# lajoiepy/cslam

Hardware: AMD Instinct MI355X
Metric: keyframes/sec (extract+match) on 100kx4096-D bank (higher is better)
Workload: dtype f32

## Files before the change

cslam_amd/csrc/conv_stem_direct_h.hip:

```cpp
#include <stdlib.h>
#include <type_traits>
#include <hip/hip_fp16.h>
#include "common.h"
#include "pairs.h"
#include "direct_dev.h"

typedef float f32x4 __attribute__((ext_vector_type(4)));
typedef unsigned u32x4 __attribute__((ext_vector_type(4)));
typedef _Float16 f16x8 __attribute__((ext_vector_type(8)));

#define SD_IW 20
#define SD_IMG (12 * SD_IW * 3)
#define SD_T9 (20 * 17)
#define SD_IMGB (SD_IMG + SD_T9)
#define SD_LDS (2 * DPATCH_BYTES + 2 * SD_IMGB * 4)

struct StemDirectArgs {
    const float *x0; const unsigned *w1; const float *b1; const float *sumw; float inv_sw1;
    const f16x8 *w2; const float *bias; float inv_sw2;
    int B, H, W, gxb, gyb, nblk;
    const unsigned *amax_in; unsigned *amax_out; float *y;
};

#ifdef CSLAM_ABLATIONS
__device__ unsigned long long *sd_prof = nullptr;
extern "C" __attribute__((visibility("default"))) int cslam_debug_sd_prof_dev(void *d_buf) {
    unsigned long long *q = (unsigned long long *)d_buf;
    return hipMemcpyToSymbol(HIP_SYMBOL(sd_prof), &q, sizeof(q)) == hipSuccess ? 0 : -2;
}
#define SD_PROF 1
#else
#define SD_PROF 0
#endif

template <bool POOL, int DBG = 0>
__global__ __launch_bounds__(256, 1) void conv_stem_direct_h_kernel(StemDirectArgs p) {
    extern __shared__ __attribute__((aligned(16))) char sd_smem[];
    const int tid = threadIdx.x;
    const int lane = tid & 63;
    const int wave = __builtin_amdgcn_readfirstlane(tid >> 6);
    const int gq = lane >> 4, l15 = lane & 15;
    unsigned *const s_img_all = (unsigned *)(sd_smem + 2 * DPATCH_BYTES);

    const float a0 = fminf(fmaxf(__uint_as_float(*p.amax_in), 1e-30f), 1e30f);
    int e_;
    (void)frexpf(16384.0f / a0, &e_);
    const float s1 = ldexpf(1.0f, e_ - 1);
    const float inv1 = p.inv_sw1 / s1;
    float bound = 0.0f;
    for (int c = 0; c < 64; ++c) bound = fmaxf(bound, fabsf(p.b1 ? p.b1[c] : 0.0f) + a0 * p.sumw[c]);
    bound = fminf(fmaxf(bound, 1e-30f), 1e30f);
    (void)frexpf(32752.0f / bound, &e_);
    const float sx = ldexpf(1.0f, e_ - 1);
    const float inv2 = p.inv_sw2 / sx;

    const DirectPart part = direct_partition(p.nblk);
    const int n_mine = part.n_mine;
    if (n_mine <= 0) return;

    f16x8 wr[9][2][2];
#pragma unroll
    for (int tap = 0; tap < 9; ++tap)
#pragma unroll
        for (int ks = 0; ks < 2; ++ks)
#pragma unroll
            for (int hl = 0; hl < 2; ++hl) {
                wr[tap][ks][hl] = p.w2[(((wave * 9 + tap) * 2 + ks) * 2 + hl) * 64 + lane];
                asm volatile("" : "+a"(wr[tap][ks][hl]));
            }
    const u32x4 w1h = ((const u32x4 *)p.w1)[(wave * 2 + 0) * 64 + lane], w1l = ((const u32x4 *)p.w1)[(wave * 2 + 1) * 64 + lane];
    const f16x8 W1h = __builtin_bit_cast(f16x8, w1h), W1l = __builtin_bit_cast(f16x8, w1l);
    const float k1 = inv1 * sx;
    float b1s[4];
#pragma unroll
    for (int r = 0; r < 4; ++r) b1s[r] = (p.b1 ? p.b1[16 * wave + 4 * gq + r] : 0.0f) * sx;
    float4 bv2;
    bv2 = p.bias ? *(const float4 *)(p.bias + 16 * wave + 4 * gq) : make_float4(0.f, 0.f, 0.f, 0.f);

    int e_dst[3], e_rc[3];
#pragma unroll
    for (int j = 0; j < 3; ++j) {
        const int e = j * 256 + tid;
        const int ci = (e >= 240) + (e >= 480);
        const int rem = e - 240 * ci;
        const int r = (rem * 3277) >> 16, c = rem - 20 * r;
        e_dst[j] = e < SD_IMG ? (r * SD_IW + c) * 3 + ci : -1;
        e_rc[j] = (ci << 16) | (r << 8) | c;
    }
    typedef DirectBlk Blk;
    auto decode_blk = [&](int bi) { return direct_decode_blk(part, bi, p.gxb, p.gyb); };
    float raw[3];
    auto img_load = [&](const Blk &b) {
#pragma unroll
        for (int j = 0; j < 3; ++j) {
            const int ci = e_rc[j] >> 16, r = (e_rc[j] >> 8) & 255, c = e_rc[j] & 255;
            const int gy = b.by * 8 - 2 + r, gx = b.bx * 16 - 2 + c;
            const bool in = (e_dst[j] >= 0) & (gy >= 0) & (gy < p.H) & (gx >= 0) & (gx < p.W);
            raw[j] = in ? p.x0[((int64_t)(b.img * 3 + ci) * p.H + gy) * p.W + gx] : 0.0f;
        }
    };
    auto img_store = [&](unsigned *s_img) {
#pragma unroll
        for (int j = 0; j < 3; ++j)
            if (e_dst[j] >= 0) {
                const unsigned v = pack_pair(raw[j] * s1);
                s_img[e_dst[j]] = v;
                if ((e_rc[j] >> 16) == 2) s_img[SD_IMG + (e_rc[j] & 255) * 17 + ((e_rc[j] >> 8) & 255)] = v;
            }
    };

    int c1_src[12], c1_dst[12];
#pragma unroll
    for (int t = 0; t < 12; ++t) {
        int pp = 16 * t + l15;
        pp = pp < DPATCH_NPIX ? pp : DPATCH_NPIX - 1;
        const int pr = (pp * 3641) >> 16, pc = pp - 18 * pr;
        c1_src[t] = (gq < 3 ? ((pr + gq) * SD_IW + pc) * 3 : SD_IMG + (pc + 2) * 17 + pr) * 4;
        c1_dst[t] = DPATCH_OFF(pr, pc, 2 * wave + (gq >> 1), gq & 1);
    }
    for (int i = tid; i < 2 * 20 * 5; i += 256)
        s_img_all[(i / 100) * SD_IMGB + SD_IMG + ((i % 100) / 5) * 17 + 12 + (i % 5)] = 0u;
    unsigned pk[2][8];
    auto conv1_read = [&](int g, const unsigned *s_img) {
#pragma unroll
        for (int i = 0; i < 2; ++i) {
            const unsigned *ib = (const unsigned *)((const char *)s_img + c1_src[2 * g + i]);
#pragma unroll
            for (int j = 0; j < 8; ++j) pk[i][j] = ib[j];
        }
    };
    f32x4 c1[2];
    float c1v[2][4];
    auto conv1_piece = [&](int g, int piece, const Blk &b, char *patch) {
        const int i = piece & 1;
        if (piece < 2) {
            u32x4 ah, al;
#pragma unroll
            for (int d = 0; d < 4; ++d) {
                ah[d] = __builtin_amdgcn_perm(pk[i][2 * d + 1], pk[i][2 * d], 0x05040100u);
                al[d] = __builtin_amdgcn_perm(pk[i][2 * d + 1], pk[i][2 * d], 0x07060302u);
            }
            const f16x8 Ph = __builtin_bit_cast(f16x8, ah), Pl = __builtin_bit_cast(f16x8, al);
            c1[i] = __builtin_amdgcn_mfma_f32_16x16x32_f16(W1l, Ph, (f32x4)(0.0f), 0, 0, 0);
            c1[i] = __builtin_amdgcn_mfma_f32_16x16x32_f16(W1h, Pl, c1[i], 0, 0, 0);
            c1[i] = __builtin_amdgcn_mfma_f32_16x16x32_f16(W1h, Ph, c1[i], 0, 0, 0);
            asm volatile("" : "+v"(c1[i]));
            return;
        }
        if (piece < 4) {
#pragma unroll
            for (int r = 0; r < 4; ++r) c1v[i][r] = fmaxf(c1[i][r] * k1 + b1s[r], 0.0f);
            return;
        }
        const __half2 h01 = __floats2half2_rn(c1v[i][0], c1v[i][1]), h23 = __floats2half2_rn(c1v[i][2], c1v[i][3]);
        const float d0 = sub_half<0>(c1v[i][0], h01), d1 = sub_half<1>(c1v[i][1], h01);
        const float d2 = sub_half<0>(c1v[i][2], h23), d3 = sub_half<1>(c1v[i][3], h23);
        const __half2 l01 = __floats2half2_rn(d0, d1), l23 = __floats2half2_rn(d2, d3);
        if ((DBG & 16) == 0 && (2 * g + i < 11 || l15 < 4)) {
            char *d = patch + c1_dst[2 * g + i];
            *(uint2 *)d = make_uint2(*(const unsigned *)&h01, *(const unsigned *)&h23);
            *(uint2 *)(d + 128) = make_uint2(*(const unsigned *)&l01, *(const unsigned *)&l23);
        }
    };
    auto border_fixup = [&](const Blk &b, char *patch) {
        const int gy0 = b.by * 8 - 1, gx0 = b.bx * 16 - 1;
        if ((gy0 >= 0) & (gy0 + 10 <= p.H) & (gx0 >= 0) & (gx0 + 18 <= p.W)) return;
#pragma unroll
        for (int k = 0; k < 3; ++k) {
            const int pp = lane + 64 * k;
            const int pr = (pp * 3641) >> 16, pc = pp - 18 * pr;
            const int gy = gy0 + pr, gx = gx0 + pc;
            if (pp < DPATCH_NPIX && !((gy >= 0) & (gy < p.H) & (gx >= 0) & (gx < p.W))) {
                char *d = patch + pr * DPATCH_RP + pc * DPATCH_PP;
                const int c0 = ((2 * wave) ^ DPATCH_SWZ(pc)) << 4, c1_ = ((2 * wave + 1) ^ DPATCH_SWZ(pc)) << 4;
                *(uint4 *)(d + c0) = make_uint4(0u, 0u, 0u, 0u); *(uint4 *)(d + c1_) = make_uint4(0u, 0u, 0u, 0u);
                *(uint4 *)(d + 128 + c0) = make_uint4(0u, 0u, 0u, 0u); *(uint4 *)(d + 128 + c1_) = make_uint4(0u, 0u, 0u, 0u);
            }
        }
    };

    float my_amax = 0.0f;
    const int Ho = POOL ? p.H >> 1 : p.H, Wo = POOL ? p.W >> 1 : p.W;
    f32x4 eacc[8];
    Blk ecb = {0, 0, 0};
    bool e_ok = false;
    auto epi_piece = [&](int k) {
        const __amdgpu_buffer_rsrc_t rsY = buf_rsrc((const char *)(p.y + (int64_t)ecb.img * Ho * Wo * 64), (int64_t)Ho * Wo * 256, RSRC_LIM16);
        const int ox = ecb.bx * 16 + l15;
        const int ch_off = (16 * wave + 4 * gq) * 4;
        if (POOL) {
            const int py = ecb.by * 4 + k;
            float4 v;
            v.x = max_f32_xor1(max_f32(eacc[2 * k][0], eacc[2 * k + 1][0])); v.y = max_f32_xor1(max_f32(eacc[2 * k][1], eacc[2 * k + 1][1]));
            v.z = max_f32_xor1(max_f32(eacc[2 * k][2], eacc[2 * k + 1][2])); v.w = max_f32_xor1(max_f32(eacc[2 * k][3], eacc[2 * k + 1][3]));
            v.x = fmaxf(v.x * inv2 + bv2.x, 0.0f); v.y = fmaxf(v.y * inv2 + bv2.y, 0.0f);
            v.z = fmaxf(v.z * inv2 + bv2.z, 0.0f); v.w = fmaxf(v.w * inv2 + bv2.w, 0.0f);
            const bool store = e_ok & ((l15 & 1) == 0) & ((ox >> 1) < Wo) & (py < Ho);
            float m = max_f32(max_f32(v.x, v.y), max_f32(v.z, v.w));
            int off = (py * Wo + (ox >> 1)) * 256 + ch_off;
            asm volatile("" : "+v"(m), "+v"(off));
            my_amax = max_f32(my_amax, store ? m : 0.0f);
            u32x4 bits;
            bits.x = __float_as_uint(v.x); bits.y = __float_as_uint(v.y); bits.z = __float_as_uint(v.z); bits.w = __float_as_uint(v.w);
            if (!(DBG & 4)) __builtin_amdgcn_raw_buffer_store_b128(bits, rsY, store ? off : 0x7fffffff, 0, 0);
        } else {
#pragma unroll
            for (int r = 2 * k; r < 2 * k + 2; ++r) {
                const int oy = ecb.by * 8 + r;
                float4 v;
                v.x = fmaxf(eacc[r][0] * inv2 + bv2.x, 0.0f); v.y = fmaxf(eacc[r][1] * inv2 + bv2.y, 0.0f);
                v.z = fmaxf(eacc[r][2] * inv2 + bv2.z, 0.0f); v.w = fmaxf(eacc[r][3] * inv2 + bv2.w, 0.0f);
                const bool store = e_ok & (ox < p.W) & (oy < p.H);
                float m = max_f32(max_f32(v.x, v.y), max_f32(v.z, v.w));
                int off = (oy * p.W + ox) * 256 + ch_off;
                asm volatile("" : "+v"(m), "+v"(off));
                my_amax = max_f32(my_amax, store ? m : 0.0f);
                u32x4 bits;
                bits.x = __float_as_uint(v.x); bits.y = __float_as_uint(v.y); bits.z = __float_as_uint(v.z); bits.w = __float_as_uint(v.w);
                __builtin_amdgcn_raw_buffer_store_b128(bits, rsY, store ? off : 0x7fffffff, 0, 0);
            }
        }
    };

    f32x4 acc[8];
    int fr_off[3];
#pragma unroll
    for (int dx = 0; dx < 3; ++dx) fr_off[dx] = DPATCH_OFF(0, l15 + dx, gq, 0);
    f16x8 fh[3], fl[3];
    auto frag_read = [&](auto col_tag, auto r_tag, const char *patch) {
        constexpr int COL = decltype(col_tag)::value, R = decltype(r_tag)::value;
        constexpr int DX = COL >> 1, KS = COL & 1, SLOT = (R + COL) % 3;
        fh[SLOT] = *(const f16x8 *)(patch + fr_off[DX] + R * DPATCH_RP + KS * 64);
        fl[SLOT] = *(const f16x8 *)(patch + fr_off[DX] + R * DPATCH_RP + KS * 64 + 128);
    };
    auto rstep = [&](auto col_tag, auto r_tag, const char *patch, const unsigned *s_img, const Blk &nblk, char *npatch) {
        constexpr int COL = decltype(col_tag)::value, R = decltype(r_tag)::value;
        constexpr int DX = COL >> 1, KS = COL & 1, SLOT = (R + COL) % 3;
        if constexpr (DBG & 2) { }
        else if constexpr (R + 2 < 10) frag_read(col_tag, std::integral_constant<int, (R + 2) % 10>{}, patch);
        else if constexpr (COL < 5) frag_read(std::integral_constant<int, (COL + 1) % 6>{}, std::integral_constant<int, (R + 2) % 10>{}, patch);
        if constexpr (R == 0 && !(DBG & 1) && !(DBG & 8)) conv1_read(COL, s_img);
#pragma unroll
        for (int prod = 0; prod < 3; ++prod)
#pragma unroll
            for (int dy = 0; dy < 3; ++dy) {
                const int r = R - dy;
                if (r < 0 || r > 7) continue;
                const f16x8 a = prod == 2 ? wr[3 * dy + DX][KS][1] : wr[3 * dy + DX][KS][0];
                const f16x8 b = prod == 1 ? fl[SLOT] : fh[SLOT];
                acc[r] = __builtin_amdgcn_mfma_f32_16x16x32_f16(a, b, (COL == 0 && prod == 0 && dy == 0) ? (f32x4)(0.0f) : acc[r], 0, 0, 0);
            }
        if constexpr (R >= 2 && R <= 7 && !(DBG & 1)) conv1_piece(COL, R - 2, nblk, npatch);
        if constexpr (COL < 2 && (R == 1 || R == 8)) epi_piece(2 * COL + (R == 8 ? 1 : 0));
        __builtin_amdgcn_sched_group_barrier(0x100, R == 0 ? 18 : 2, 0);
        constexpr int NM = 3 * ((R < 2 ? R + 1 : 3) - (R > 7 ? R - 7 : 0)) + ((R == 2 || R == 3) ? 3 : 0);
#pragma unroll
        for (int m = 0; m < NM; ++m) {
            __builtin_amdgcn_sched_group_barrier(0x008, 1, 0);
            __builtin_amdgcn_sched_group_barrier(0x002, (COL < 2 && (R == 1 || R == 8)) ? 6 : 3, 0);
        }
        __builtin_amdgcn_sched_group_barrier(0x200, 2, 0);
        __builtin_amdgcn_sched_barrier(0);
    };
    auto edge = [&](auto col_tag, const char *patch, const unsigned *s_img) {
        constexpr int COL = decltype(col_tag)::value;
        constexpr int DX = COL >> 1, KS = COL & 1, SLOT = (9 + COL) % 3;
        constexpr int DX2 = (COL + 1) >> 1, KS2 = (COL + 1) & 1, SLOT2 = (COL + 1) % 3;
        if constexpr (!(DBG & 2)) frag_read(std::integral_constant<int, COL + 1>{}, std::integral_constant<int, 1>{}, patch);
        if constexpr (!(DBG & 1) && !(DBG & 8)) conv1_read(COL + 1, s_img);
#pragma unroll
        for (int prod = 0; prod < 3; ++prod) {
            acc[7] = __builtin_amdgcn_mfma_f32_16x16x32_f16(prod == 2 ? wr[6 + DX][KS][1] : wr[6 + DX][KS][0], prod == 1 ? fl[SLOT] : fh[SLOT], acc[7], 0, 0, 0);
            acc[0] = __builtin_amdgcn_mfma_f32_16x16x32_f16(prod == 2 ? wr[DX2][KS2][1] : wr[DX2][KS2][0], prod == 1 ? fl[SLOT2] : fh[SLOT2], acc[0], 0, 0, 0);
        }
        if constexpr (!(DBG & 2)) frag_read(std::integral_constant<int, COL + 1>{}, std::integral_constant<int, 2>{}, patch);
        __builtin_amdgcn_sched_group_barrier(0x100, 10, 0);
#pragma unroll
        for (int m = 0; m < 6; ++m) {
            __builtin_amdgcn_sched_group_barrier(0x008, 1, 0);
            __builtin_amdgcn_sched_group_barrier(0x002, 3, 0);
        }
        __builtin_amdgcn_sched_barrier(0);
    };
    auto column = [&](auto col_tag, const char *patch, const unsigned *s_img, const Blk &nblk, char *npatch) {
        constexpr int COL_ = decltype(col_tag)::value;
        if constexpr (COL_ == 0) rstep(col_tag, std::integral_constant<int, 0>{}, patch, s_img, nblk, npatch);
        rstep(col_tag, std::integral_constant<int, 1>{}, patch, s_img, nblk, npatch);
        rstep(col_tag, std::integral_constant<int, 2>{}, patch, s_img, nblk, npatch); rstep(col_tag, std::integral_constant<int, 3>{}, patch, s_img, nblk, npatch);
        rstep(col_tag, std::integral_constant<int, 4>{}, patch, s_img, nblk, npatch); rstep(col_tag, std::integral_constant<int, 5>{}, patch, s_img, nblk, npatch);
        rstep(col_tag, std::integral_constant<int, 6>{}, patch, s_img, nblk, npatch); rstep(col_tag, std::integral_constant<int, 7>{}, patch, s_img, nblk, npatch);
        rstep(col_tag, std::integral_constant<int, 8>{}, patch, s_img, nblk, npatch);
        if constexpr (COL_ == 5) rstep(col_tag, std::integral_constant<int, 9>{}, patch, s_img, nblk, npatch);
        else edge(col_tag, patch, s_img);
    };
#define SD_C(T) std::integral_constant<int, T>{}

    [[maybe_unused]] unsigned long long t_main = 0, t_epi = 0, t_bar = 0, t1 = 0, t2 = 0, t3 = 0;
    Blk cb = decode_blk(0);
    img_load(cb);
    img_store(s_img_all);
    Blk nb = decode_blk(1);
    img_load(nb);
    __syncthreads();
#pragma unroll
    for (int g = 0; g < 6; ++g) {
        conv1_read(g, s_img_all);
#pragma unroll
        for (int piece = 0; piece < 6; ++piece) conv1_piece(g, piece, cb, sd_smem);
        __builtin_amdgcn_sched_barrier(0);
    }
    border_fixup(cb, sd_smem);
    img_store(s_img_all + SD_IMGB);
    __syncthreads();
    for (int bi = 0; bi < n_mine; ++bi) {
        const int cur = bi & 1;
        const char *const patch = sd_smem + cur * DPATCH_BYTES;
        char *const npatch = sd_smem + (cur ^ 1) * DPATCH_BYTES;
        const unsigned *const s_img_next = s_img_all + (cur ^ 1) * SD_IMGB;
        const Blk nnb = decode_blk(bi + 2);
        img_load(nnb);
        if (SD_PROF) t1 = __builtin_amdgcn_s_memtime();
        frag_read(SD_C(0), SD_C(0), patch);
        frag_read(SD_C(0), SD_C(1), patch);
        column(SD_C(0), patch, s_img_next, nb, npatch); column(SD_C(1), patch, s_img_next, nb, npatch); column(SD_C(2), patch, s_img_next, nb, npatch);
        column(SD_C(3), patch, s_img_next, nb, npatch); column(SD_C(4), patch, s_img_next, nb, npatch); column(SD_C(5), patch, s_img_next, nb, npatch);
        if (!(DBG & 1)) border_fixup(nb, npatch);
        if (SD_PROF) { t2 = __builtin_amdgcn_s_memtime(); t_main += t2 - t1; }
        img_store(s_img_all + cur * SD_IMGB);
#pragma unroll
        for (int r = 0; r < 8; ++r) eacc[r] = acc[r];
        ecb = cb;
        e_ok = true;
        if (SD_PROF) { t3 = __builtin_amdgcn_s_memtime(); t_epi += t3 - t2; }
        __syncthreads();
        if (SD_PROF) t_bar += __builtin_amdgcn_s_memtime() - t3;
        cb = nb;
        nb = nnb;
    }
#pragma unroll
    for (int k = 0; k < 4; ++k) epi_piece(k);
#ifdef CSLAM_ABLATIONS
    if (sd_prof && blockIdx.x == 0 && tid == 0) { sd_prof[0] = t_main; sd_prof[1] = t_epi; sd_prof[2] = t_bar; sd_prof[3] = 0; sd_prof[4] = (unsigned long long)n_mine; }
#endif

    if (p.amax_out) {
        __syncthreads();
        amax_publish(my_amax, p.amax_out, sd_smem, tid, lane);
    }
}

CSLAM_API int cslam_conv_stem_direct_h_dev(const float *d_x0, const void *d_w1, const float *d_b1, const float *d_sumw, float inv_sw1,
                                           const void *d_w2r, const float *d_bias, float inv_sw2, int B, int H, int W, int pool,
                                           const unsigned *d_amax_x0, unsigned *d_amax_out, float *d_y, void *stream) {
    PTR_DEVICE(d_x0);
    ARG_CHECK(d_x0 && d_w1 && d_sumw && d_w2r && d_y && d_amax_x0, "NULL argument");
    ARG_CHECK(B >= 1 && H >= 1 && W >= 1, "empty map");
    ARG_CHECK(!pool || ((H % 2) == 0 && (W % 2) == 0), "pooling needs even H and W");
    ARG_CHECK(inv_sw1 > 0.0f && inv_sw2 > 0.0f, "scales must be positive");
    ARG_CHECK((int64_t)H * W * 256 < 0x7ffffff0ll, "one image's output map must stay below 2 GiB (32-bit buffer offsets)");
    StemDirectArgs a;
    a.x0 = d_x0; a.w1 = (const unsigned *)d_w1; a.b1 = d_b1; a.sumw = d_sumw; a.inv_sw1 = inv_sw1;
    a.w2 = (const f16x8 *)d_w2r; a.bias = d_bias; a.inv_sw2 = inv_sw2;
    a.B = B; a.H = H; a.W = W;
    a.gxb = (int)ceil_div64(W, 16); a.gyb = (int)ceil_div64(H, 8);
    const int64_t nblk = (int64_t)B * a.gxb * a.gyb;
    ARG_CHECK(nblk < (1ll << 30), "too many blocks for one launch");
    a.nblk = (int)nblk;
    a.amax_in = d_amax_x0; a.amax_out = d_amax_out; a.y = d_y;
    const int n_cu = cslam_cu_count();
    ARG_CHECK(n_cu > 0, "no HIP device");
    const int grid = (int)(nblk < n_cu ? nblk : n_cu);
    hipStream_t st = (hipStream_t)stream;
    const dim3 g(grid), b(256);
#ifdef CSLAM_ABLATIONS
    if (const char *e = getenv("CSLAM_SD_DBG")) {
        const int d = atoi(e);
        if (d == 1) return launch_lds<conv_stem_direct_h_kernel<true, 1>>(g, b, SD_LDS, st, a);
        if (d == 2) return launch_lds<conv_stem_direct_h_kernel<true, 2>>(g, b, SD_LDS, st, a);
        if (d == 3) return launch_lds<conv_stem_direct_h_kernel<true, 3>>(g, b, SD_LDS, st, a);
        if (d == 4) return launch_lds<conv_stem_direct_h_kernel<true, 4>>(g, b, SD_LDS, st, a);
        if (d == 7) return launch_lds<conv_stem_direct_h_kernel<true, 7>>(g, b, SD_LDS, st, a);
        if (d == 8) return launch_lds<conv_stem_direct_h_kernel<true, 8>>(g, b, SD_LDS, st, a);
        if (d == 16) return launch_lds<conv_stem_direct_h_kernel<true, 16>>(g, b, SD_LDS, st, a);
        if (d == 24) return launch_lds<conv_stem_direct_h_kernel<true, 24>>(g, b, SD_LDS, st, a);
    }
#endif
    if (pool) return launch_lds<conv_stem_direct_h_kernel<true>>(g, b, SD_LDS, st, a);
    return launch_lds<conv_stem_direct_h_kernel<false>>(g, b, SD_LDS, st, a);
}
```

cslam_amd/csrc/direct_dev.h:

```cpp
#pragma once
#include <hip/hip_fp16.h>
#include "common.h"
#include "pairs.h"

typedef unsigned dd_u32x2 __attribute__((ext_vector_type(2)));
typedef unsigned dd_u32x4 __attribute__((ext_vector_type(4)));
typedef float dd_f32x2 __attribute__((ext_vector_type(2)));

struct DirectPart { int wg_j, wg_per, blk_beg, blk_cnt, n_mine, half; };
template <bool PAIRS = false>
__device__ __forceinline__ DirectPart direct_partition(int nblk) {
    DirectPart q;
    const bool by_xcd = (gridDim.x & (PAIRS ? 15 : 7)) == 0;
    const int wg_xcd = by_xcd ? (int)blockIdx.x & 7 : 0, wg_raw = by_xcd ? (int)blockIdx.x >> 3 : (int)blockIdx.x;
    q.half = PAIRS ? wg_raw & 1 : 0;
    q.wg_j = PAIRS ? wg_raw >> 1 : wg_raw;
    q.wg_per = (by_xcd ? (int)gridDim.x >> 3 : (int)gridDim.x) >> (PAIRS ? 1 : 0);
    const int per_xcd = by_xcd ? (nblk + 7) >> 3 : nblk;
    q.blk_beg = wg_xcd * per_xcd;
    q.blk_cnt = min(per_xcd, nblk - q.blk_beg);
    q.n_mine = q.blk_cnt > q.wg_j ? (q.blk_cnt - q.wg_j + q.wg_per - 1) / q.wg_per : 0;
    return q;
}

struct DirectBlk { int img, by, bx; };
__device__ __forceinline__ DirectBlk direct_decode_blk(const DirectPart &q, int bi, int gxb, int gyb) {
    int blk = q.wg_j + bi * q.wg_per;
    blk = q.blk_beg + (blk < q.blk_cnt ? blk : q.blk_cnt - 1);
    const int per_img = gxb * gyb;
    DirectBlk b;
    b.img = blk / per_img;
    const int rem = blk - b.img * per_img;
    b.by = rem / gxb; b.bx = rem - b.by * gxb;
    return b;
}

__device__ __forceinline__ void amax_publish(float &my_amax, unsigned *amax_out, void *lds_slot, int tid, int lane) {
    unsigned *s_amax = (unsigned *)lds_slot;
    if (tid == 0) *s_amax = 0u;
    __syncthreads();
#pragma unroll
    for (int o = 32; o > 0; o >>= 1) my_amax = fmaxf(my_amax, __shfl_xor(my_amax, o, 64));
    if (lane == 0) atomicMax(s_amax, __float_as_uint(my_amax));
    __syncthreads();
    if (tid == 0 && *s_amax > *(volatile unsigned *)amax_out) atomicMax(amax_out, *s_amax);
}

constexpr int DPATCH_PP = 320;
constexpr int DPATCH_RP = 18 * DPATCH_PP;
constexpr int DPATCH_BYTES = 10 * DPATCH_RP;
constexpr int DPATCH_NPIX = 180;
constexpr int DPATCH_LO = 128;
#define DPATCH_SWZ(pc) (((pc) >> 1) & 3)
#define DPATCH_OFF(pr, pc, chunk, q) ((pr) * DPATCH_RP + (pc) * DPATCH_PP + (((chunk) ^ DPATCH_SWZ(pc)) << 4) + (q) * 8)

template <class Dst>
__device__ __forceinline__ void dpatch_split_store(dd_u32x4 v, float s, Dst dst) {
    dd_f32x2 w01 = dd_f32x2{__uint_as_float(v.x), __uint_as_float(v.y)} * dd_f32x2{s, s};
    dd_f32x2 w23 = dd_f32x2{__uint_as_float(v.z), __uint_as_float(v.w)} * dd_f32x2{s, s};
    asm("" : "+v"(w01), "+v"(w23));
    const __half2 h01 = __floats2half2_rn(w01[0], w01[1]), h23 = __floats2half2_rn(w23[0], w23[1]);
    const float d0 = sub_half<0>(w01[0], h01), d1 = sub_half<1>(w01[1], h01), d2 = sub_half<0>(w23[0], h23), d3 = sub_half<1>(w23[1], h23);
    const __half2 l01 = __floats2half2_rn(d0, d1), l23 = __floats2half2_rn(d2, d3);
    char *d = dst();
    *(uint2 *)d = make_uint2(*(const unsigned *)&h01, *(const unsigned *)&h23);
    *(uint2 *)(d + DPATCH_LO) = make_uint2(*(const unsigned *)&l01, *(const unsigned *)&l23);
// ... 14 lines not shown
```

cslam_amd/vpr/conv_kernels.py:

```python
import torch

from .. import _lib
from .heads import _p, _stream


def _po(t):
    return _p(t) if t is not None else None


def _out(B, C, H, W, pool, device):
    Ho, Wo = (H // 2, W // 2) if pool else (H, W)
    return torch.empty((B, C, Ho, Wo), dtype=torch.float32, device=device, memory_format=torch.channels_last)


def _amax_slot(x, slot, have=False):
    if not have and x.numel() % 4 == 0:
        _lib.check(_lib.load().cslam_absmax_dev(_p(x), x.numel(), _p(slot), _stream(x)))
    elif not have:
        slot.copy_(x.abs().max().reshape(1))
    return slot


def stem_pool_fits(Ho, Wo):
    return Ho % 8 == 0 and Wo % 16 == 0
# ... 100 lines not shown
    y = _out(B, 128, H, W, pool, x.device)
    _lib.check(fn(_p(x), _p(Wr[0]), _po(bias), B, H, W, Cin, 128, int(relu), int(pool), _p(amax_in), float(Wr[1]), _po(amax_out),
                  _p(y), _stream(x)))
    return y


def conv3x3_direct_r(x, Wr, bias, relu, pool, amax_in, amax_out=None):
    return _direct_r(_lib.load().cslam_conv3x3_direct_r_dev, x, Wr, bias, relu, pool, amax_in, amax_out)


def conv3x3_direct_r2(x, Wr2, bias, relu, pool, amax_in, amax_out=None):
    return _direct_r(_lib.load().cslam_conv3x3_direct_r2_dev, x, Wr2, bias, relu, pool, amax_in, amax_out)


def conv3x3_direct_r_pairs(x, Wr, bias, wl1, bmax, amax_in, bound_out, amax_out=None):
    x = x.contiguous(memory_format=torch.channels_last)
    B, Cin, H, W = x.shape
    y = torch.empty((B, H, W, 4, 2, 32), dtype=torch.float16, device=x.device)
    _lib.check(_lib.load().cslam_conv3x3_direct_r_pairs_dev(_p(x), _p(Wr[0]), _po(bias), B, H, W, Cin, 128, _p(amax_in), float(Wr[1]),
                                                            float(wl1), float(bmax), _po(amax_out), _p(bound_out), _p(y), _stream(x)))
    return y


def conv3x3_direct_hp(xp, shape, bound, Wd, bias, relu, pool, amax_out=None):
    B, Cin, H, W = shape
    W2, inv_sw = Wd
    Cout = W2.shape[1]
    y = _out(B, Cout, H, W, pool, xp.device)
    _lib.check(_lib.load().cslam_conv3x3_direct_hp_dev(_p(xp), _p(bound), _p(W2), _po(bias), B, H, W, Cin, Cout, int(relu), int(pool),
                                                       float(inv_sw), _po(amax_out), _p(y), _stream(xp)))
    return y


def conv_stem_direct_h(x0, stem, bias1, Wr, bias, pool, amax_x0, amax_out=None):
    B, C3, H, W = x0.shape
    assert C3 == 3 and x0.is_contiguous()
    y = _out(B, 64, H, W, pool, x0.device)
    _lib.check(_lib.load().cslam_conv_stem_direct_h_dev(
        _p(x0), _p(stem[0]), _po(bias1), _p(stem[2]), float(stem[1]), _p(Wr[0]), _po(bias), float(Wr[1]), B, H, W, int(pool),
        _p(amax_x0), _po(amax_out), _p(y), _stream(x0)))
    return y


def wino_stem64_h(x0, stem, bias1, Uh, bias, pool, amax_x0, amax_out=None):
    B, C3, H, W = x0.shape
    assert C3 == 3 and x0.is_contiguous() and Uh[0].shape[2] == 4
    y = _out(B, 64, H, W, pool, x0.device)
    _lib.check(_lib.load().cslam_wino4_stem_c64_h_dev(
        _p(x0), _p(stem[0]), _po(bias1), _p(stem[2]), float(stem[1]), _p(Uh[0]), _po(bias), B, H, W, int(pool), _p(amax_x0),
        float(Uh[1]), _po(amax_out), _p(y), _stream(x0)))
    return y


def _residual_like(residual, y):
    if residual is not None:
        residual = residual.contiguous(memory_format=torch.channels_last)
        assert residual.shape == y.shape
    return residual


def wino_fused64_h(x, Uh, bias, relu, pool, amax_in, amax_out=None, residual=None):
    B, _, H, W = x.shape
    Cout = Uh[0].shape[2] * 16
    y = _out(B, Cout, H, W, pool, x.device)
    residual = _residual_like(residual, y)
    _lib.check(_lib.load().cslam_wino4_fused_c64_h_dev(
        _p(x), _p(Uh[0]), _po(bias), _po(residual), B, H, W, Cout, int(relu), int(pool), _p(amax_in), float(Uh[1]), _po(amax_out),
        _p(y), _stream(x)))
    return y


def wino_fused64(x, Up, bias, relu, pool, residual=None):
    lib = _lib.load()
# ... 8 lines not shown
```

cslam_amd/vpr/winograd.py:

```python
import os

import torch
from torch import nn

from .. import _lib
from .conv_kernels import (PairAct, _amax_slot, _out, _po, _residual_like, conv3x3_direct_h, conv3x3_direct_hp,
                           conv3x3_direct_p, conv3x3_direct_r, conv3x3_direct_r2, conv3x3_direct_r_pairs, conv_igemm, conv_igemm_p,
                           conv_stem_direct_h, direct_p_fits, pairs_to_float, stem_pool_fits, wino_fused64, wino_fused64_h,
                           wino_stem64_h)
from .heads import _p, _stream
from .pair_weights import (direct_pair_weights, direct_r2_pair_weights, direct_r_pair_weights, fused64_pair_weights,
                           fused64_weights, igemm_pair_weights, out_bound, split16_pair_weights, split16_weights,
                           stem_direct_pair_weights, stem_pair_weights, wino_weights)


def _pair(v):
    return tuple(v) if isinstance(v, (tuple, list)) else (v, v)


_TUNED = {"done": False}


def use_tuned_gemms():
    if _TUNED["done"] or os.environ.get("CSLAM_TUNED_GEMM", "1") == "0" or not torch.cuda.is_available():
# ... 230 lines not shown
            for b in self.blocks:
                idt = cur if b["down"] is None else runp(b["down"], cur, False, None)
                o = runp(b["c1"], cur, True, None)
                if b["c3"] is None:
                    cur = runp(b["c2"], o, True, idt)
                else:
                    o = runp(b["c2"], o, True, None)
                    cur = runp(b["c3"], o, True, idt)
            return cur.t
        for b in self.blocks:
            idt = x if b["down"] is None else run(b["down"], x, False, None, ax)[0]
            o, ao = run(b["c1"], x, True, None, ax)
            if b["c3"] is None:
                x, ax = run(b["c2"], o, True, idt, ao)
            else:
                o, ao = run(b["c2"], o, True, None, ao)
                x, ax = run(b["c3"], o, True, idt, ao)
        return x


class _Step(object):
    __slots__ = ("kind", "module", "conv", "relu", "pool", "U", "U4", "U3", "U2", "Up", "Uph", "bias", "stem", "Wd", "Wr", "Wdr", "Wdr2", "wl1", "bmax")

    def __init__(self):
        for name in self.__slots__:
            setattr(self, name, None)
        self.kind, self.relu, self.pool = "torch", False, False


def _wants(st):
    return st.U3 is not None or st.U2 is not None or st.Uph is not None or st.Wd is not None


TRUNK_FORMS = {"conv_direct": 1, "conv_direct_r": True, "conv_direct_r2": True, "stem_direct": True, "wino_stem": True, "fused_h": True, "split16_min_cin": None,
               "wino_chain": True}
CHAIN_TILE_COLS = (5, 16)
FP32_GEMM_FORMS = {"split16_min_cin": 0, "fused_h": False, "wino_stem": False}


def _pool2_at(mods, i):
    p = mods[i] if i < len(mods) else None
    return (isinstance(p, nn.MaxPool2d) and p.kernel_size in (2, (2, 2)) and p.stride in (2, (2, 2))
            and p.padding in (0, (0, 0)) and not p.ceil_mode)


class WinogradTrunk(_Workspace):

    def __init__(self, encoder, min_in_channels=256, tile=2, fused64=None, split16_h3=False, forms=None):
        super().__init__()
        self.encoder = encoder
        self.min_in_channels = int(min_in_channels)
        self.tile = int(tile)
        self.fused64 = True if fused64 is None else bool(fused64)
        self.fused_min_blocks = 256
        self.fused_couts = (64, 128)
        self.input_bound = None
        self.forms = dict(TRUNK_FORMS)
        self.forms.update(forms or {})
        assert set(self.forms) == set(TRUNK_FORMS), "unknown trunk form"
        self.direct128 = int(self.forms["conv_direct"]) != 0
        self.direct_cins = (128,) if int(self.forms["conv_direct"]) == 2 else (64, 128)
        self.split16_h3 = bool(split16_h3)
        self.split16_min_cin = (256 if self.split16_h3 else 128) if self.forms["split16_min_cin"] is None else int(self.forms["split16_min_cin"])
        use_tuned_gemms()
        self.refresh()

    def refresh(self):
# ... 65 lines not shown
                    a.stem = stem_pair_weights(a.conv.weight)
                    if self.forms["stem_direct"]:
                        a.Wr = stem_direct_pair_weights(b.conv.weight)
        return self

    def _chain_len(self, k, B, H, W):
        if not (self.forms["wino_chain"] and _f4_fits(B, H, W) and CHAIN_TILE_COLS[0] <= -(-W // 4) <= CHAIN_TILE_COLS[1]):
            return 1
        pair = lambda st_: (st_.kind == "wino" and st_.U2 is not None and st_.Wd is None and st_.Up is None
                            and not _z_form(st_.conv.in_channels, st_.conv.out_channels))
        n = 1
        while (k + n < len(self.steps) and pair(self.steps[k + n - 1]) and pair(self.steps[k + n])
               and self.steps[k + n - 1].relu and not self.steps[k + n - 1].pool):
            n += 1
        return n

    def _want(self, slots, j):
        return slots[j:j + 1] if j < len(self.steps) and _wants(self.steps[j]) else None


    def _stem_pair(self, k, x, slots):
        st, (B, _, H, W) = self.steps[k], x.shape
        nxt = self.steps[k + 1] if st.stem is not None else None
        if nxt is None or not (B * -(-H // 16) * -(-W // 16) >= self.fused_min_blocks and not (nxt.pool and (H % 2 or W % 2))
                               and B * H * W * 64 < 2 ** 31):
            return None
        slot = slots[k:k + 1]
        if self.input_bound is not None:
            slot.fill_(float(self.input_bound))
        else:
            _amax_slot(x, slot)
        want = self._want(slots, k + 2)
        if st.Wr is not None:
            y = conv_stem_direct_h(x, st.stem, st.bias, st.Wr, nxt.bias, nxt.pool, slot, want)
        else:
            y = wino_stem64_h(x, st.stem, st.bias, nxt.Uph, nxt.bias, nxt.pool, slot, want)
        return y, want is not None, 1

    def _first_layer(self, k, x, slots):
        st, (B, _, H, W) = self.steps[k], x.shape
        Cout = st.conv.out_channels
        y = _out(B, Cout, H, W, False, x.device)
        want = self._want(slots, k + 1) if Cout == 64 else None
        _lib.check(_lib.load().cslam_conv3x3_c3_amax_dev(_p(x), _p(st.U), _po(st.bias), B, H, W, Cout, int(st.relu), _p(y), _po(want),
                                                         _stream(x)))
        return y, want is not None, 0

    def _torch_direct(self, k, x):
        st = self.steps[k]
        c = st.conv
        x = torch.nn.functional.conv2d(x, c.weight, None, c.stride, c.padding, c.dilation)
        x = x.contiguous(memory_format=torch.channels_last)
        B, Cout, H, W = x.shape
        pool = st.pool and H % 2 == 0 and W % 2 == 0
        y = _out(B, Cout, H, W, True, x.device) if pool else x
        _lib.check(_lib.load().cslam_bias_act_pool_dev(_p(x), _p(st.bias), B, H, W, Cout, 1, int(pool), _p(y), _stream(x)))
        return (torch.nn.functional.max_pool2d(y, 2, 2) if st.pool and not pool else y), None, 0

    def _direct128(self, k, x, have, slots):
        st, (B, _, H, W) = self.steps[k], x.shape
        if not (st.Wd is not None and not (st.pool and (H % 2 or W % 2))
                and B * -(-H // 16) * -(-W // 16) >= self.fused_min_blocks and x.numel() % 4 == 0):
            return None
        slot = _amax_slot(x, slots[k:k + 1], have)
        nxt = self.steps[k + 1] if k + 1 < len(self.steps) else None
        if (VGG_PAIRS and st.Wdr is not None and st.relu and not st.pool and nxt is not None and nxt.Wd is not None
                and nxt.Wdr is None and nxt.conv.in_channels == 128 and H * W * 512 < 2 ** 31 - 16
# ... 66 lines not shown
```

Measured before the change: 19240.

## Walk stem blocks in vertical strips and carry overlapping conv1 halo rows

The fused stem kernel now gives each workgroup a contiguous run of blocks ordered down columns (strip partition), so consecutive blocks are vertically adjacent. Instead of recomputing all 10 conv1 patch rows per block, it copies the bottom two rows of the current patch into the next patch buffer and computes only the 8 new rows, with head rows recomputed at strip starts. This cuts redundant conv1 MFMA work and image reads, at the cost of extra LDS carry traffic, changed scheduling barriers, and a coarser per-XCD split that may hurt load balance.

```diff
diff --git a/cslam_amd/csrc/conv_stem_direct_h.hip b/cslam_amd/csrc/conv_stem_direct_h.hip
--- a/cslam_amd/csrc/conv_stem_direct_h.hip
+++ b/cslam_amd/csrc/conv_stem_direct_h.hip
@@ -14,11 +14,12 @@
 #define SD_T9 (20 * 17)
 #define SD_IMGB (SD_IMG + SD_T9)
 #define SD_LDS (2 * DPATCH_BYTES + 2 * SD_IMGB * 4)
+#define SD_CARRY (2 * DPATCH_RP / 16)
 
 struct StemDirectArgs {
     const float *x0; const unsigned *w1; const float *b1; const float *sumw; float inv_sw1;
     const f16x8 *w2; const float *bias; float inv_sw2;
-    int B, H, W, gxb, gyb, nblk;
+    int B, H, W, gxb, gyb, nblk, reuse;
     const unsigned *amax_in; unsigned *amax_out; float *y;
 };
 
@@ -54,7 +55,7 @@
     const float sx = ldexpf(1.0f, e_ - 1);
     const float inv2 = p.inv_sw2 / sx;
 
-    const DirectPart part = direct_partition(p.nblk);
+    const StripPart part = strip_partition(p.nblk);
     const int n_mine = part.n_mine;
     if (n_mine <= 0) return;
 
@@ -88,7 +89,7 @@
         e_rc[j] = (ci << 16) | (r << 8) | c;
     }
     typedef DirectBlk Blk;
-    auto decode_blk = [&](int bi) { return direct_decode_blk(part, bi, p.gxb, p.gyb); };
+    auto decode_blk = [&](int bi) { return strip_decode_blk(part, bi, p.gxb, p.gyb); };
     float raw[3];
     auto img_load = [&](const Blk &b) {
 #pragma unroll
@@ -109,31 +110,32 @@
             }
     };
 
-    int c1_src[12], c1_dst[12];
-#pragma unroll
-    for (int t = 0; t < 12; ++t) {
-        int pp = 16 * t + l15;
-        pp = pp < DPATCH_NPIX ? pp : DPATCH_NPIX - 1;
-        const int pr = (pp * 3641) >> 16, pc = pp - 18 * pr;
-        c1_src[t] = (gq < 3 ? ((pr + gq) * SD_IW + pc) * 3 : SD_IMG + (pc + 2) * 17 + pr) * 4;
+    int c1_src[9], c1_dst[9];
+    auto c1_src_of = [&](int pr, int pc) { return (gq < 3 ? ((pr + gq) * SD_IW + pc) * 3 : SD_IMG + (pc + 2) * 17 + pr) * 4; };
+#pragma unroll
+    for (int t = 0; t < 9; ++t) {
+        const int pp = 16 * t + l15;
+        const int q = (pp * 3641) >> 16;
+        const int pr = 2 + q, pc = pp - 18 * q;
+        c1_src[t] = c1_src_of(pr, pc);
         c1_dst[t] = DPATCH_OFF(pr, pc, 2 * wave + (gq >> 1), gq & 1);
     }
     for (int i = tid; i < 2 * 20 * 5; i += 256)
         s_img_all[(i / 100) * SD_IMGB + SD_IMG + ((i % 100) / 5) * 17 + 12 + (i % 5)] = 0u;
     unsigned pk[2][8];
+    auto conv1_read1 = [&](int i, int src, const unsigned *s_img) {
+        const unsigned *ib = (const unsigned *)((const char *)s_img + src);
+#pragma unroll
+        for (int j = 0; j < 8; ++j) pk[i][j] = ib[j];
+    };
     auto conv1_read = [&](int g, const unsigned *s_img) {
-#pragma unroll
-        for (int i = 0; i < 2; ++i) {
-            const unsigned *ib = (const unsigned *)((const char *)s_img + c1_src[2 * g + i]);
-#pragma unroll
-            for (int j = 0; j < 8; ++j) pk[i][j] = ib[j];
-        }
+        conv1_read1(0, c1_src[3 * (g >> 1) + 2 * (g & 1)], s_img);
+        if ((g & 1) == 0) conv1_read1(1, c1_src[3 * (g >> 1) + 1], s_img);
     };
     f32x4 c1[2];
     float c1v[2][4];
-    auto conv1_piece = [&](int g, int piece, const Blk &b, char *patch) {
-        const int i = piece & 1;
-        if (piece < 2) {
+    auto conv1_tile = [&](int kind, int i, char *d) {
+        if (kind == 0) {
             u32x4 ah, al;
 #pragma unroll
             for (int d = 0; d < 4; ++d) {
@@ -147,7 +149,7 @@
             asm volatile("" : "+v"(c1[i]));
             return;
         }
-        if (piece < 4) {
+        if (kind == 1) {
 #pragma unroll
             for (int r = 0; r < 4; ++r) c1v[i][r] = fmaxf(c1[i][r] * k1 + b1s[r], 0.0f);
             return;
@@ -156,27 +158,41 @@
         const float d0 = sub_half<0>(c1v[i][0], h01), d1 = sub_half<1>(c1v[i][1], h01);
         const float d2 = sub_half<0>(c1v[i][2], h23), d3 = sub_half<1>(c1v[i][3], h23);
         const __half2 l01 = __floats2half2_rn(d0, d1), l23 = __floats2half2_rn(d2, d3);
-        if ((DBG & 16) == 0 && (2 * g + i < 11 || l15 < 4)) {
-            char *d = patch + c1_dst[2 * g + i];
+        if ((DBG & 16) == 0) {
             *(uint2 *)d = make_uint2(*(const unsigned *)&h01, *(const unsigned *)&h23);
             *(uint2 *)(d + 128) = make_uint2(*(const unsigned *)&l01, *(const unsigned *)&l23);
         }
     };
-    auto border_fixup = [&](const Blk &b, char *patch) {
+    auto border_fixup = [&](const Blk &b, char *patch, int pp_lo, int pp_hi) {
         const int gy0 = b.by * 8 - 1, gx0 = b.bx * 16 - 1;
         if ((gy0 >= 0) & (gy0 + 10 <= p.H) & (gx0 >= 0) & (gx0 + 18 <= p.W)) return;
 #pragma unroll
         for (int k = 0; k < 3; ++k) {
-            const int pp = lane + 64 * k;
+            const int pp = pp_lo + lane + 64 * k;
             const int pr = (pp * 3641) >> 16, pc = pp - 18 * pr;
             const int gy = gy0 + pr, gx = gx0 + pc;
-            if (pp < DPATCH_NPIX && !((gy >= 0) & (gy < p.H) & (gx >= 0) & (gx < p.W))) {
+            if (pp < pp_hi && !((gy >= 0) & (gy < p.H) & (gx >= 0) & (gx < p.W))) {
                 char *d = patch + pr * DPATCH_RP + pc * DPATCH_PP;
                 const int c0 = ((2 * wave) ^ DPATCH_SWZ(pc)) << 4, c1_ = ((2 * wave + 1) ^ DPATCH_SWZ(pc)) << 4;
                 *(uint4 *)(d + c0) = make_uint4(0u, 0u, 0u, 0u); *(uint4 *)(d + c1_) = make_uint4(0u, 0u, 0u, 0u);
                 *(uint4 *)(d + 128 + c0) = make_uint4(0u, 0u, 0u, 0u); *(uint4 *)(d + 128 + c1_) = make_uint4(0u, 0u, 0u, 0u);
             }
         }
+    };
+
+    auto head_rows = [&](const Blk &b, char *patch, const unsigned *s_img) {
+#pragma unroll
+        for (int t = 0; t < 3; ++t) {
+            int pp = 16 * t + l15;
+            pp = pp < 36 ? pp : 35;
+            const int pr = pp >= 18 ? 1 : 0, pc = pp - 18 * pr;
+            conv1_read1(0, c1_src_of(pr, pc), s_img);
+            conv1_tile(0, 0, nullptr);
+            conv1_tile(1, 0, nullptr);
+            conv1_tile(2, 0, patch + DPATCH_OFF(pr, pc, 2 * wave + (gq >> 1), gq & 1));
+        }
+        border_fixup(b, patch, 0, 36);
+        __syncthreads();
     };
 
     float my_amax = 0.0f;
@@ -227,18 +243,30 @@
 #pragma unroll
     for (int dx = 0; dx < 3; ++dx) fr_off[dx] = DPATCH_OFF(0, l15 + dx, gq, 0);
     f16x8 fh[3], fl[3];
-    auto frag_read = [&](auto col_tag, auto r_tag, const char *patch) {
+    const char *patch = sd_smem;
+    char *npatch = sd_smem + DPATCH_BYTES;
+    const int cy_off = tid * 16, cy_off2 = (tid + 512 < SD_CARRY ? tid + 512 : SD_CARRY - 1) * 16;
+    u32x4 cy[3];
+    auto carry_read = [&]() {
+        cy[0] = *(const u32x4 *)(patch + 8 * DPATCH_RP + cy_off); cy[1] = *(const u32x4 *)(patch + 8 * DPATCH_RP + cy_off + 4096);
+        cy[2] = *(const u32x4 *)(patch + 8 * DPATCH_RP + cy_off2);
+    };
+    auto carry_write = [&]() {
+        *(u32x4 *)(npatch + cy_off) = cy[0]; *(u32x4 *)(npatch + cy_off + 4096) = cy[1];
+        *(u32x4 *)(npatch + cy_off2) = cy[2];
+    };
+    auto frag_read = [&](auto col_tag, auto r_tag) {
         constexpr int COL = decltype(col_tag)::value, R = decltype(r_tag)::value;
         constexpr int DX = COL >> 1, KS = COL & 1, SLOT = (R + COL) % 3;
         fh[SLOT] = *(const f16x8 *)(patch + fr_off[DX] + R * DPATCH_RP + KS * 64);
         fl[SLOT] = *(const f16x8 *)(patch + fr_off[DX] + R * DPATCH_RP + KS * 64 + 128);
     };
-    auto rstep = [&](auto col_tag, auto r_tag, const char *patch, const unsigned *s_img, const Blk &nblk, char *npatch) {
+    auto rstep = [&](auto col_tag, auto r_tag, const unsigned *s_img) {
         constexpr int COL = decltype(col_tag)::value, R = decltype(r_tag)::value;
         constexpr int DX = COL >> 1, KS = COL & 1, SLOT = (R + COL) % 3;
         if constexpr (DBG & 2) { }
-        else if constexpr (R + 2 < 10) frag_read(col_tag, std::integral_constant<int, (R + 2) % 10>{}, patch);
-        else if constexpr (COL < 5) frag_read(std::integral_constant<int, (COL + 1) % 6>{}, std::integral_constant<int, (R + 2) % 10>{}, patch);
+        else if constexpr (R + 2 < 10) frag_read(col_tag, std::integral_constant<int, (R + 2) % 10>{});
+        else if constexpr (COL < 5) frag_read(std::integral_constant<int, (COL + 1) % 6>{}, std::integral_constant<int, (R + 2) % 10>{});
         if constexpr (R == 0 && !(DBG & 1) && !(DBG & 8)) conv1_read(COL, s_img);
 #pragma unroll
         for (int prod = 0; prod < 3; ++prod)
@@ -250,30 +278,36 @@
                 const f16x8 b = prod == 1 ? fl[SLOT] : fh[SLOT];
                 acc[r] = __builtin_amdgcn_mfma_f32_16x16x32_f16(a, b, (COL == 0 && prod == 0 && dy == 0) ? (f32x4)(0.0f) : acc[r], 0, 0, 0);
             }
-        if constexpr (R >= 2 && R <= 7 && !(DBG & 1)) conv1_piece(COL, R - 2, nblk, npatch);
+        constexpr int T0 = 3 * (COL >> 1) + 2 * (COL & 1);
+        if constexpr (R >= 2 && R <= 7 && !(DBG & 1)) {
+            if constexpr ((COL & 1) == 0) conv1_tile((R - 2) >> 1, (R - 2) & 1, npatch + c1_dst[T0 + ((R - 2) & 1)]);
+            else if constexpr ((R & 1) == 0) conv1_tile((R - 2) >> 1, 0, npatch + c1_dst[T0]);
+        }
+        if constexpr (COL == 3 && R == 3) carry_read();
+        if constexpr (COL == 5 && R == 3) carry_write();
         if constexpr (COL < 2 && (R == 1 || R == 8)) epi_piece(2 * COL + (R == 8 ? 1 : 0));
-        __builtin_amdgcn_sched_group_barrier(0x100, R == 0 ? 18 : 2, 0);
-        constexpr int NM = 3 * ((R < 2 ? R + 1 : 3) - (R > 7 ? R - 7 : 0)) + ((R == 2 || R == 3) ? 3 : 0);
+        __builtin_amdgcn_sched_group_barrier(0x100, R == 0 ? 18 : (COL == 3 && R == 3) ? 5 : 2, 0);
+        constexpr int NM = 3 * ((R < 2 ? R + 1 : 3) - (R > 7 ? R - 7 : 0)) + ((R == 2 || (R == 3 && (COL & 1) == 0)) ? 3 : 0);
 #pragma unroll
         for (int m = 0; m < NM; ++m) {
             __builtin_amdgcn_sched_group_barrier(0x008, 1, 0);
             __builtin_amdgcn_sched_group_barrier(0x002, (COL < 2 && (R == 1 || R == 8)) ? 6 : 3, 0);
         }
-        __builtin_amdgcn_sched_group_barrier(0x200, 2, 0);
+        __builtin_amdgcn_sched_group_barrier(0x200, (COL == 5 && R == 3) ? 3 : 2, 0);
         __builtin_amdgcn_sched_barrier(0);
     };
-    auto edge = [&](auto col_tag, const char *patch, const unsigned *s_img) {
+    auto edge = [&](auto col_tag, const unsigned *s_img) {
         constexpr int COL = decltype(col_tag)::value;
         constexpr int DX = COL >> 1, KS = COL & 1, SLOT = (9 + COL) % 3;
         constexpr int DX2 = (COL + 1) >> 1, KS2 = (COL + 1) & 1, SLOT2 = (COL + 1) % 3;
-        if constexpr (!(DBG & 2)) frag_read(std::integral_constant<int, COL + 1>{}, std::integral_constant<int, 1>{}, patch);
+        if constexpr (!(DBG & 2)) frag_read(std::integral_constant<int, COL + 1>{}, std::integral_constant<int, 1>{});
         if constexpr (!(DBG & 1) && !(DBG & 8)) conv1_read(COL + 1, s_img);
 #pragma unroll
         for (int prod = 0; prod < 3; ++prod) {
             acc[7] = __builtin_amdgcn_mfma_f32_16x16x32_f16(prod == 2 ? wr[6 + DX][KS][1] : wr[6 + DX][KS][0], prod == 1 ? fl[SLOT] : fh[SLOT], acc[7], 0, 0, 0);
             acc[0] = __builtin_amdgcn_mfma_f32_16x16x32_f16(prod == 2 ? wr[DX2][KS2][1] : wr[DX2][KS2][0], prod == 1 ? fl[SLOT2] : fh[SLOT2], acc[0], 0, 0, 0);
         }
-        if constexpr (!(DBG & 2)) frag_read(std::integral_constant<int, COL + 1>{}, std::integral_constant<int, 2>{}, patch);
+        if constexpr (!(DBG & 2)) frag_read(std::integral_constant<int, COL + 1>{}, std::integral_constant<int, 2>{});
         __builtin_amdgcn_sched_group_barrier(0x100, 10, 0);
 #pragma unroll
         for (int m = 0; m < 6; ++m) {
@@ -282,16 +316,16 @@
         }
         __builtin_amdgcn_sched_barrier(0);
     };
-    auto column = [&](auto col_tag, const char *patch, const unsigned *s_img, const Blk &nblk, char *npatch) {
+    auto column = [&](auto col_tag, const unsigned *s_img) {
         constexpr int COL_ = decltype(col_tag)::value;
-        if constexpr (COL_ == 0) rstep(col_tag, std::integral_constant<int, 0>{}, patch, s_img, nblk, npatch);
-        rstep(col_tag, std::integral_constant<int, 1>{}, patch, s_img, nblk, npatch);
-        rstep(col_tag, std::integral_constant<int, 2>{}, patch, s_img, nblk, npatch); rstep(col_tag, std::integral_constant<int, 3>{}, patch, s_img, nblk, npatch);
-        rstep(col_tag, std::integral_constant<int, 4>{}, patch, s_img, nblk, npatch); rstep(col_tag, std::integral_constant<int, 5>{}, patch, s_img, nblk, npatch);
-        rstep(col_tag, std::integral_constant<int, 6>{}, patch, s_img, nblk, npatch); rstep(col_tag, std::integral_constant<int, 7>{}, patch, s_img, nblk, npatch);
-        rstep(col_tag, std::integral_constant<int, 8>{}, patch, s_img, nblk, npatch);
-        if constexpr (COL_ == 5) rstep(col_tag, std::integral_constant<int, 9>{}, patch, s_img, nblk, npatch);
-        else edge(col_tag, patch, s_img);
+        if constexpr (COL_ == 0) rstep(col_tag, std::integral_constant<int, 0>{}, s_img);
+        rstep(col_tag, std::integral_constant<int, 1>{}, s_img);
+        rstep(col_tag, std::integral_constant<int, 2>{}, s_img); rstep(col_tag, std::integral_constant<int, 3>{}, s_img);
+        rstep(col_tag, std::integral_constant<int, 4>{}, s_img); rstep(col_tag, std::integral_constant<int, 5>{}, s_img);
+        rstep(col_tag, std::integral_constant<int, 6>{}, s_img); rstep(col_tag, std::integral_constant<int, 7>{}, s_img);
+        rstep(col_tag, std::integral_constant<int, 8>{}, s_img);
+        if constexpr (COL_ == 5) rstep(col_tag, std::integral_constant<int, 9>{}, s_img);
+        else edge(col_tag, s_img);
     };
 #define SD_C(T) std::integral_constant<int, T>{}
 
@@ -303,28 +337,30 @@
     img_load(nb);
     __syncthreads();
 #pragma unroll
-    for (int g = 0; g < 6; ++g) {
-        conv1_read(g, s_img_all);
-#pragma unroll
-        for (int piece = 0; piece < 6; ++piece) conv1_piece(g, piece, cb, sd_smem);
+    for (int t = 0; t < 9; ++t) {
+        conv1_read1(0, c1_src[t], s_img_all);
+        conv1_tile(0, 0, nullptr);
+        conv1_tile(1, 0, nullptr);
+        conv1_tile(2, 0, sd_smem + c1_dst[t]);
         __builtin_amdgcn_sched_barrier(0);
     }
-    border_fixup(cb, sd_smem);
+    border_fixup(cb, sd_smem, 36, DPATCH_NPIX);
     img_store(s_img_all + SD_IMGB);
     __syncthreads();
     for (int bi = 0; bi < n_mine; ++bi) {
         const int cur = bi & 1;
-        const char *const patch = sd_smem + cur * DPATCH_BYTES;
-        char *const npatch = sd_smem + (cur ^ 1) * DPATCH_BYTES;
         const unsigned *const s_img_next = s_img_all + (cur ^ 1) * SD_IMGB;
         const Blk nnb = decode_blk(bi + 2);
         img_load(nnb);
+        patch = sd_smem + cur * DPATCH_BYTES;
+        npatch = sd_smem + (cur ^ 1) * DPATCH_BYTES;
+        if ((bi == 0) | (cb.by == 0) | (p.reuse == 0)) head_rows(cb, sd_smem + cur * DPATCH_BYTES, s_img_all + cur * SD_IMGB);
         if (SD_PROF) t1 = __builtin_amdgcn_s_memtime();
-        frag_read(SD_C(0), SD_C(0), patch);
-        frag_read(SD_C(0), SD_C(1), patch);
-        column(SD_C(0), patch, s_img_next, nb, npatch); column(SD_C(1), patch, s_img_next, nb, npatch); column(SD_C(2), patch, s_img_next, nb, npatch);
-        column(SD_C(3), patch, s_img_next, nb, npatch); column(SD_C(4), patch, s_img_next, nb, npatch); column(SD_C(5), patch, s_img_next, nb, npatch);
-        if (!(DBG & 1)) border_fixup(nb, npatch);
+        frag_read(SD_C(0), SD_C(0));
+        frag_read(SD_C(0), SD_C(1));
+        column(SD_C(0), s_img_next); column(SD_C(1), s_img_next); column(SD_C(2), s_img_next);
+        column(SD_C(3), s_img_next); column(SD_C(4), s_img_next); column(SD_C(5), s_img_next);
+        if (!(DBG & 1)) border_fixup(nb, npatch, 36, DPATCH_NPIX);
         if (SD_PROF) { t2 = __builtin_amdgcn_s_memtime(); t_main += t2 - t1; }
         img_store(s_img_all + cur * SD_IMGB);
 #pragma unroll
@@ -362,6 +398,8 @@
     a.x0 = d_x0; a.w1 = (const unsigned *)d_w1; a.b1 = d_b1; a.sumw = d_sumw; a.inv_sw1 = inv_sw1;
     a.w2 = (const f16x8 *)d_w2r; a.bias = d_bias; a.inv_sw2 = inv_sw2;
     a.B = B; a.H = H; a.W = W;
+    a.reuse = (pool & 2) ? 0 : 1;
+    pool &= 1;
     a.gxb = (int)ceil_div64(W, 16); a.gyb = (int)ceil_div64(H, 8);
     const int64_t nblk = (int64_t)B * a.gxb * a.gyb;
     ARG_CHECK(nblk < (1ll << 30), "too many blocks for one launch");
diff --git a/cslam_amd/csrc/direct_dev.h b/cslam_amd/csrc/direct_dev.h
--- a/cslam_amd/csrc/direct_dev.h
+++ b/cslam_amd/csrc/direct_dev.h
@@ -32,6 +32,31 @@
     b.img = blk / per_img;
     const int rem = blk - b.img * per_img;
     b.by = rem / gxb; b.bx = rem - b.by * gxb;
+    return b;
+}
+
+struct StripPart { int blk_beg, n_mine; };
+__device__ __forceinline__ StripPart strip_partition(int nblk) {
+    StripPart q;
+    const bool by_xcd = (gridDim.x & 7) == 0;
+    const int wg_xcd = by_xcd ? (int)blockIdx.x & 7 : 0, wg_j = by_xcd ? (int)blockIdx.x >> 3 : (int)blockIdx.x;
+    const int wg_per = by_xcd ? (int)gridDim.x >> 3 : (int)gridDim.x;
+    const int per_xcd = by_xcd ? (nblk + 7) >> 3 : nblk;
+    const int xcd_beg = wg_xcd * per_xcd;
+    const int cnt = max(min(per_xcd, nblk - xcd_beg), 0);
+    const int r0 = (int)((int64_t)wg_j * cnt / wg_per), r1 = (int)((int64_t)(wg_j + 1) * cnt / wg_per);
+    q.blk_beg = xcd_beg + r0;
+    q.n_mine = r1 - r0;
+    return q;
+}
+
+__device__ __forceinline__ DirectBlk strip_decode_blk(const StripPart &q, int bi, int gxb, int gyb) {
+    const int blk = q.blk_beg + (bi < q.n_mine ? bi : q.n_mine - 1);
+    const int per_img = gxb * gyb;
+    DirectBlk b;
+    b.img = blk / per_img;
+    const int rem = blk - b.img * per_img;
+    b.bx = rem / gyb; b.by = rem - b.bx * gyb;
     return b;
 }
 
diff --git a/cslam_amd/vpr/conv_kernels.py b/cslam_amd/vpr/conv_kernels.py
--- a/cslam_amd/vpr/conv_kernels.py
+++ b/cslam_amd/vpr/conv_kernels.py
@@ -156,13 +156,13 @@
     return y
 
 
-def conv_stem_direct_h(x0, stem, bias1, Wr, bias, pool, amax_x0, amax_out=None):
+def conv_stem_direct_h(x0, stem, bias1, Wr, bias, pool, amax_x0, amax_out=None, strips=True):
     B, C3, H, W = x0.shape
     assert C3 == 3 and x0.is_contiguous()
     y = _out(B, 64, H, W, pool, x0.device)
     _lib.check(_lib.load().cslam_conv_stem_direct_h_dev(
-        _p(x0), _p(stem[0]), _po(bias1), _p(stem[2]), float(stem[1]), _p(Wr[0]), _po(bias), float(Wr[1]), B, H, W, int(pool),
-        _p(amax_x0), _po(amax_out), _p(y), _stream(x0)))
+        _p(x0), _p(stem[0]), _po(bias1), _p(stem[2]), float(stem[1]), _p(Wr[0]), _po(bias), float(Wr[1]), B, H, W,
+        int(bool(pool)) | (0 if strips else 2), _p(amax_x0), _po(amax_out), _p(y), _stream(x0)))
     return y
 
 
diff --git a/cslam_amd/vpr/winograd.py b/cslam_amd/vpr/winograd.py
--- a/cslam_amd/vpr/winograd.py
+++ b/cslam_amd/vpr/winograd.py
@@ -286,7 +286,7 @@
     return st.U3 is not None or st.U2 is not None or st.Uph is not None or st.Wd is not None
 
 
-TRUNK_FORMS = {"conv_direct": 1, "conv_direct_r": True, "conv_direct_r2": True, "stem_direct": True, "wino_stem": True, "fused_h": True, "split16_min_cin": None,
+TRUNK_FORMS = {"conv_direct": 1, "conv_direct_r": True, "conv_direct_r2": True, "stem_direct": True, "stem_strips": True, "wino_stem": True, "fused_h": True, "split16_min_cin": None,
                "wino_chain": True}
 CHAIN_TILE_COLS = (5, 16)
 FP32_GEMM_FORMS = {"split16_min_cin": 0, "fused_h": False, "wino_stem": False}
@@ -418,7 +418,7 @@
             _amax_slot(x, slot)
         want = self._want(slots, k + 2)
         if st.Wr is not None:
-            y = conv_stem_direct_h(x, st.stem, st.bias, st.Wr, nxt.bias, nxt.pool, slot, want)
+            y = conv_stem_direct_h(x, st.stem, st.bias, st.Wr, nxt.bias, nxt.pool, slot, want, bool(self.forms["stem_strips"]))
         else:
             y = wino_stem64_h(x, st.stem, st.bias, nxt.Uph, nxt.bias, nxt.pool, slot, want)
         return y, want is not None, 1
```

After: 19360, median of 5. No clear change (+0.7%).
